# haosulab/ActiveZero

Hardware: AMD Instinct MI355X
Metric: stereo pairs/sec (540x960, D=192) fwd+bwd (higher is better)
Workload: dtype f32; 1 GPU; configs[1]: PSMNet 540x960 (padded to 544 rows) D=192 fwd+bwd+Adam, supervised disparity loss, batch 4 per GPU; global_batch=4, height=540, width=960, maxdisp=192, parallelism=dp1

## Files before the change

### activezero_amd/agg3d.py

```python
import torch

from . import bn2d, conv3d, costconv, ops


def _mode_of(conv):
    if isinstance(conv, torch.nn.ConvTranspose3d):
        return conv3d.DECONV_S2
    return conv3d.CONV_S1 if conv.stride[0] == 1 else conv3d.CONV_S2


def volume_from_features(feat_l, feat_r, ndisp, lazy=None):
    fl = feat_l.permute(0, 2, 3, 1).contiguous()
    fr = feat_r.permute(0, 2, 3, 1).contiguous()
    if lazy is None:
        lazy = not torch.is_grad_enabled()
    if lazy:
        return conv3d.LazyCostVolume(fl, fr, ndisp)
    return ops.cost_volume_ndhwc(fl, fr, ndisp)


def costvol_conv_bn(feat_l, feat_r, ndisp, unit, relu=False, arith=None):
    conv, bn = unit[0], unit[1]
    raw = costconv.costvol_conv(feat_l, feat_r, ndisp, conv.weight, arith)
    b, d, h, w, c = raw.shape
    y = bn2d.bn_act(raw.view(b, d * h, w, c).permute(0, 3, 1, 2), bn, relu=relu)
    return y.permute(0, 2, 3, 1).reshape(b, d, h, w, c)


def conv_bn(vol, unit, relu=False, add=None, arith=None, defer=None):
    return conv3d.conv_bn(vol, unit[0], unit[1], _mode_of(unit[0]), relu, add, arith, defer)


def deconv_bn(vol, unit, relu=False, add=None, arith=None):
    return conv3d.conv_bn(vol, unit[0], unit[1], conv3d.DECONV_S2, relu, add, arith)


def conv_logits(vol, conv, add=None, arith=None, affine=None):
    return conv3d.conv_logits(vol, conv, add, arith.sink if arith is not None else None, affine)


def add(a, b):
    return conv3d.add(a, b)


def fanout(x, n):
    return conv3d.fanout(x, n)
```

### activezero_amd/conv3d.py

```python
import collections
import os

import torch

from . import _lib, overlap, packing, profiler
from .amax import AMAX_SLOTS, ZEROS, absmax, _get_amax, _set_amax, weight_amax
from .handover import slot_contribute, slot_leftover, slot_register, sum_parts
from .ops import _call, _chk, _p, _stream

CONV_S1, CONV_S2, DECONV_S2 = 0, 1, 2
FP32, BF16X6, F16X3 = 0, 1, 3
_PREC = {"fp32": FP32, "bf16x6": BF16X6, "f16x3": F16X3}
_BWD_F16 = os.environ.get("AZ_BWD_F16", "1") != "0"
PRESPLIT = os.environ.get("AZ_PRESPLIT", "1") != "0"
BF16X6_R16 = 2
_ROLL = os.environ.get("AZ_CONV_ROLL", "1") != "0"


_OFF32 = 0xffffff00


def _fits32(x, cin, cout):
    if isinstance(x, LazyCostVolume):
        return True
# ... 322 lines not shown
    return _wgrad(dy, x, 1 if mode == CONV_S1 else 2, cout, cin, "conv", precision, sink)


def _presplit_ok(x, raw, mode, cin, cout, need_gx, need_gw):
    lib = _lib.lib()
    b, d, h, w, _ = raw.shape
    if need_gx:
        op, ci, co = _dgrad_launch(mode, cin, cout)[:3]
        if not _f16_launch_ok(op, ci, co, raw) or lib.az_conv3d_fwd_f16_split_ok(op, b, ci, co, d, h, w) != 1:
            return False
    if need_gw:
        if not _f16_wgrad_ok(mode, cin, cout):
            return False
        _, dx_, hx, wx, _ = x.shape
        if mode == DECONV_S2:
            ok, bit = lib.az_conv3d_wgrad_f16_split_ok(2, b, cin, cout, dx_, hx, wx, d, h, w), 2
        else:
            ok, bit = lib.az_conv3d_wgrad_f16_split_ok(1 if mode == CONV_S1 else 2, b, cout, cin, d, h, w, dx_, hx, wx), 1
        if not ok & bit:
            return False
    return bool(need_gx or need_gw)


class _ConvBN(torch.autograd.Function):

    @staticmethod
    def forward(ctx, x, weight, gamma, beta, residual, bn, mode, relu, arith, defer=None, x_slot=None, res_slot=None):
        ctx.x_slot, ctx.res_slot = x_slot, res_slot
        x = _chk(x, "x")
        if residual is not None:
            residual = _chk(residual, "residual")
        training = bn.training or not bn.track_running_stats
        eps = float(bn.eps)
        cin, cout = _fwd_launch(weight, mode)[:2]
        with torch.cuda.device(x.device):
            if not training:
                scale, shift = eval_affine(bn, x)
                raw = _conv(x, weight, mode, arith.conv)
                y = torch.empty_like(raw)
                y_amax = ZEROS.take(raw)
                _call("az_bn3d_apply", _p(y), _p(raw), _p(scale), _p(shift), _p(residual), int(relu),
                      raw.numel() // cout, cout, _p(y_amax), _stream())
                _set_amax(y, y_amax)
                ctx.save_for_backward(x, weight, gamma, raw, y if relu else None, bn.running_mean.clone(),
                                      scale, None, None)
                ctx.cfg = (mode, relu, residual is not None, cin, cout, arith, False)
                return y
            raw, part, cnt, ntiles = _conv(x, weight, mode, arith.conv, stats=True)
            scale, shift = x.new_empty(cout), x.new_empty(cout)
            mean, invstd = x.new_empty(cout), x.new_empty(cout)
            track = bn.track_running_stats and bn.running_mean is not None
            momentum = 0.1 if bn.momentum is None else float(bn.momentum)
            nbt = bn.num_batches_tracked if (track and bn.num_batches_tracked is not None) else None
            scratch = x.new_empty(int(_lib.lib().az_bn3d_finalize_scratch(cout))) if ntiles >= 4096 else None
            _call("az_bn3d_finalize", _p(mean), _p(invstd), _p(scale), _p(shift),
                  _p(bn.running_mean) if track else None, _p(bn.running_var) if track else None,
                  _p(part), _p(cnt), _p(gamma.detach()), _p(beta.detach()), ntiles, cout, eps,
                  momentum, _p(nbt), _p(scratch), scratch.numel() if scratch is not None else 0, _stream())
            if nbt is not None:
                packing.touched(nbt, bn.running_mean, bn.running_var)
            nvox = raw.numel() // cout
            if defer is not None and relu and residual is None:
                defer.scale, defer.shift = scale, shift
                y = raw
            else:
                y = torch.empty_like(raw)
                y_amax = ZEROS.take(raw)
                with profiler.scope(f"bn3d_apply_{cout}", bytes=4.0 * raw.numel() * (3 if residual is not None else 2),
                                    bound="hbm"):
                    _call("az_bn3d_apply", _p(y), _p(raw), _p(scale), _p(shift), _p(residual), int(relu),
                          nvox, cout, _p(y_amax), _stream())
                _set_amax(y, y_amax)
        remask = relu and residual is None
        ctx.save_for_backward(x, weight, gamma, raw, y if (relu and not remask) else None, mean, invstd,
                              scale if remask else None, shift if remask else None)
        if arith.sink is not None and not arith.sink.owns(weight):
            arith = arith._replace(sink=None)
        ctx.cfg = (mode, relu, residual is not None, cin, cout, arith, True)
        ctx.x_amax = _get_amax(x)
        return y

    @staticmethod
    def backward(ctx, gy):
# ... 11 lines not shown
                dgamma = (dz * (raw - rm)).sum(dim=(0, 1, 2, 3)) * rinv
                dx_raw = (dz * s_).contiguous()
                g_res = dz if has_res else None
            else:
                lib = _lib.lib()
                dx_raw = torch.empty_like(raw)
                dz = torch.empty_like(raw) if (has_res and relu) else None
                dgamma, dbeta = gy.new_empty(cout), gy.new_empty(cout)
                coef = gy.new_empty(cout, 3)
                ws_bytes = lib.az_bn3d_bwd_workspace(nvox, cout)
                ws = gy.new_empty(ws_bytes // 4)
                dx_amax = gy.new_empty(AMAX_SLOTS) if arith.bwd16 else None
                split = arith.bwd16 and PRESPLIT and _presplit_ok(x, raw, mode, cin, cout, ctx.needs_input_grad[0],
                                                                  ctx.needs_input_grad[1])
                with profiler.scope(f"bn3d_bwd_{cout}", bytes=4.0 * raw.numel() * (7 if (relu and y is not None) else 5), bound="hbm"):
                    _call("az_bn3d_bwd", _p(dx_raw), _p(dz), _p(dgamma), _p(dbeta), _p(coef), _p(ws), ws_bytes,
                          _p(gy), _p(y), _p(raw), _p(mean), _p(invstd), _p(gamma.detach()), _p(scale), _p(shift),
                          int(relu), nvox, cout, _p(dx_amax), int(split), _stream())
                if dx_amax is not None:
                    _set_amax(dx_raw, dx_amax)
                if split:
                    dx_raw.az_split = True
                g_res = (dz if relu else gy) if has_res else None
            gx = gw = None
            if has_res:
                g_res = slot_contribute(ctx.res_slot, plain=g_res)
            if ctx.needs_input_grad[0]:
                gx = slot_contribute(ctx.x_slot, make=lambda r: _input_grad(dx_raw, weight, mode, cin, cout,
                                                                             F16X3 if arith.bwd16 else arith.conv, r))
            if ctx.needs_input_grad[1]:
                if getattr(ctx, "x_amax", None) is not None and _get_amax(x) is None:
                    _set_amax(x, ctx.x_amax)
                gw = _weight_grad(x, dx_raw, mode, cin, cout, F16X3 if arith.bwd16 else arith.wgrad, arith.sink)
        return gx, gw, dgamma, dbeta, g_res, None, None, None, None, None, None, None


class DeferredAffine:

    def __init__(self):
        self.scale = self.shift = None

    @property
    def pending(self):
        return self.scale is not None


def conv_bn(x, conv, bn, mode, relu=False, residual=None, arith=None, defer=None):
    arith = _arith(arith)
    if isinstance(x, LazyCostVolume):
        if torch.is_grad_enabled() or bn.training:
            raise RuntimeError("LazyCostVolume is an inference-only operand")
        with torch.cuda.device(x.fl.device):
            scale, shift = eval_affine(bn, x.fl, cache=True)
            return _conv(x, conv.weight, mode, arith.conv, scale, shift, residual, relu, cache=True)
    training = bn.training or not bn.track_running_stats
    if not training and not torch.is_grad_enabled():
# ... 32 lines not shown
    def backward(ctx, g):
        x, w, scale, shift = ctx.saved_tensors
        g = _chk(g.contiguous(), "grad_logits")
        b, d, h, wd, _ = _dims(x)
        gx = gw = None
        with torch.cuda.device(g.device):
            if ctx.needs_input_grad[0]:
                gx = torch.empty_like(x)
                with profiler.scope("conv3d_c1_dgrad", bytes=4.0 * (x.numel() + g.numel()), bound="hbm"):
                    _call("az_conv3d_c1_dgrad", _p(gx), _p(g), _p(w), b, d, h, wd, _stream())
            if ctx.needs_input_grad[1]:
                gw = torch.empty_like(w)
                with overlap.scope(ctx.sink, x, g, gw, scale, shift), \
                        profiler.scope("conv3d_c1_wgrad", bytes=4.0 * (x.numel() + g.numel()), bound="hbm"):
                    _call("az_conv3d_c1_wgrad", _p(gw), _p(x), _p(g), _p(scale), _p(shift), b, d, h, wd, _stream())
        return gx, gw, (g if ctx.has_add else None), None, None, None


def conv_logits(x, conv, addend=None, sink=None, affine=None):
    sc, sh = (affine.scale, affine.shift) if (affine is not None and affine.pending) else (None, None)
    return _ConvLogits.apply(x, sink.weight(conv.weight) if sink is not None else conv.weight, addend, sink, sc, sh)


class _AddRelu(torch.autograd.Function):
    @staticmethod
    def forward(ctx, a, b):
        a, b = _chk(a, "a"), _chk(b, "b")
        y = torch.empty_like(a)
        y_amax = ZEROS.take(a)
        with torch.cuda.device(a.device):
            _call("az_add_relu", _p(y), _p(a), _p(b), 0, a.numel(), _p(y_amax), _stream())
        _set_amax(y, y_amax)
        return y

    @staticmethod
    def backward(ctx, g):
        return g, g


def add(a, b):
    return _AddRelu.apply(a, b)


class _FanOut(torch.autograd.Function):

    @staticmethod
# ... 27 lines not shown
```

### activezero_amd/csrc/az_conv3d_c1.hip

```cpp
#include "az_common.h"
#include "az_launch_math.h"

#define C1_TH 8
#define C1_TW 32
#define C1_VS 36
#define C1_GP 36
typedef float c1_f2 __attribute__((ext_vector_type(2)));
#define C1_FMA2(a, b, c) __builtin_elementwise_fma(a, b, c)


#define C1F_TH 8
#define C1F_TW 16
template <int CTRL>
__device__ __forceinline__ float c1_dpp_add(float v) {
    return v + __builtin_bit_cast(float, __builtin_amdgcn_update_dpp(0, __builtin_bit_cast(int, v), CTRL, 0xf, 0xf, true));
}
__global__ void __launch_bounds__(256)
c1_fwd_kernel(float *__restrict__ out, const float *__restrict__ in, const float *__restrict__ w,
              const float *__restrict__ addend, const float *__restrict__ in_scale,
              const float *__restrict__ in_shift, int D, int H, int W, int tiles_x, int dseg) {
    constexpr int SX = C1F_TW + 2, SY = C1F_TH + 2;
    __shared__ __attribute__((aligned(16))) float slab[SY * SX * C1_VS];
    const int tx0 = (blockIdx.x % tiles_x) * C1F_TW, ty0 = (blockIdx.x / tiles_x) * C1F_TH;
    const int d0 = blockIdx.y * dseg, d1 = min(d0 + dseg, D), b = blockIdx.z;
// ... 70 lines not shown
        const int od = id - 1;
        if (od >= d0 && od < d1) {
            float mine = 0.f;
#pragma unroll
            for (int j = 0; j < 8; ++j) {
                float v = a_prev[j][0] + a_prev[j][1];
                v = c1_dpp_add<0xB1>(v);
                v = c1_dpp_add<0x4E>(v);
                v = c1_dpp_add<0x141>(v);
                v = c1_dpp_add<0x140>(v);
                mine = (cp == j) ? v : mine;
            }
            const int ow = tx0 + lx0 + cp;
            if (cp < 8 && oh < H && ow < W) {
                const size_t o = (((size_t)b * D + od) * H + oh) * W + ow;
                out[o] = addend ? mine + addend[o] : mine;
            }
        }
#pragma unroll
        for (int j = 0; j < 8; ++j) { a_prev[j] = a_cur[j]; a_cur[j] = a_next[j]; a_next[j] = c1_f2{0.f, 0.f}; }
    }
}

__device__ __forceinline__ void c1_load_gtile(float *gt, const float *__restrict__ gout, int b,
                                              int od, int ty0, int tx0, int D, int H, int W) {
    constexpr int SX = C1_TW + 2, SY = C1_TH + 2;
    for (int q = threadIdx.x; q < 3 * SY * SX; q += 256) {
        const int sx = q % SX;
        const int r = q / SX;
        const int sy = r % SY, sd = r / SY;
        const int gd = od - 1 + sd, gh = ty0 - 1 + sy, gw = tx0 - 1 + sx;
        gt[r * C1_GP + sx] = (gd >= 0 && gd < D && gh >= 0 && gh < H && gw >= 0 && gw < W)
                                 ? gout[(((size_t)b * D + gd) * H + gh) * W + gw] : 0.f;
    }
}
__device__ __forceinline__ void c1_row6(float (&r)[6], const float *gt, int pd, int sy, int lx0) {
    const float *row = static_cast<const float *>(__builtin_assume_aligned(gt + (pd * (C1_TH + 2) + sy) * C1_GP + lx0, 16));
    const float4 a = *reinterpret_cast<const float4 *>(row);
    const float2 c = *reinterpret_cast<const float2 *>(row + 4);
    r[0] = a.x; r[1] = a.y; r[2] = a.z; r[3] = a.w; r[4] = c.x; r[5] = c.y;
}

__global__ void __launch_bounds__(256)
c1_dgrad_kernel(float *__restrict__ gin, const float *__restrict__ gout,
                const float *__restrict__ w, int D, int H, int W, int tiles_x) {
    constexpr int SY = C1_TH + 2;
    __shared__ __attribute__((aligned(16))) float gt[3 * SY * C1_GP];
    const int tx0 = (blockIdx.x % tiles_x) * C1_TW, ty0 = (blockIdx.x / tiles_x) * C1_TH;
    const int od = blockIdx.y, b = blockIdx.z;
    c1_load_gtile(gt, gout, b, od, ty0, tx0, D, H, W);
    const int cp = threadIdx.x & 15, grp = threadIdx.x >> 4;
    c1_f2 wp[27];
#pragma unroll
    for (int t = 0; t < 27; ++t) wp[t] = c1_f2{w[(cp * 2 + 0) * 27 + t], w[(cp * 2 + 1) * 27 + t]};
    __syncthreads();
#pragma unroll 1
    for (int p = 0; p < C1_TH * C1_TW / 128; ++p) {
// ... 94 lines not shown
                        const int t = (kd * 3 + kh) * 3 + kw;
#pragma unroll
                        for (int j = 0; j < 4; ++j) {
                            const c1_f2 g2 = {r[j + 2 - kw], r[j + 2 - kw]};
                            a01[t] = C1_FMA2(g2, x01[j], a01[t]);
                            a23[t] = C1_FMA2(g2, x23[j], a23[t]);
                        }
                    }
                }
        }
    }
#pragma unroll
    for (int c = 0; c < 4; ++c)
#pragma unroll
        for (int t = 0; t < 27; ++t) {
            float v = (c < 2 ? a01[t] : a23[t])[c & 1];
            v += __shfl_xor(v, 8); v += __shfl_xor(v, 16); v += __shfl_xor(v, 32);
            if ((threadIdx.x & 63) < 8) atomicAdd(&red[(quad * 4 + c) * 27 + t], v);
        }
    __syncthreads();
    for (int q = threadIdx.x; q < 864; q += 256) atomicAdd(&gw[q], red[q]);
}

static int c1_check(int B, int D, int H, int W) {
    if (!(B > 0 && D > 0 && H > 0 && W > 0)) return AZ_EINVAL;
    if (B > 65535 || D > 65535) return AZ_EUNSUPPORTED;
    return AZ_OK;
}

extern "C" int az_conv3d_c1_fwd(float *logits, const float *in, const float *w,
                                const float *addend, const float *in_scale, const float *in_shift, int B, int D,
                                int H, int W, void *stream) {
    AZ_REQUIRE_PTR(logits); AZ_REQUIRE_PTR(in); AZ_REQUIRE_PTR(w);
    if ((in_scale == nullptr) != (in_shift == nullptr)) return AZ_EINVAL;
    if (int e = c1_check(B, D, H, W)) return e;
    const int tiles_x = (W + C1F_TW - 1) / C1F_TW, tiles_y = (H + C1F_TH - 1) / C1F_TH;
    const int best = az_c1_fwd_dseg((long long)tiles_x * tiles_y * B, D);
    hipLaunchKernelGGL(c1_fwd_kernel, dim3(tiles_x * tiles_y, (D + best - 1) / best, B), dim3(256), 0,
                       az_stream(stream), logits, in, w, addend, in_scale, in_shift, D, H, W, tiles_x, best);
    return az_launch_status();
}

extern "C" int az_conv3d_c1_dgrad(float *grad_in, const float *grad_logits, const float *w,
                                  int B, int D, int H, int W, void *stream) {
    AZ_REQUIRE_PTR(grad_in); AZ_REQUIRE_PTR(grad_logits); AZ_REQUIRE_PTR(w);
    if (int e = c1_check(B, D, H, W)) return e;
    const int tiles_x = (W + C1_TW - 1) / C1_TW, tiles_y = (H + C1_TH - 1) / C1_TH;
    hipLaunchKernelGGL(c1_dgrad_kernel, dim3(tiles_x * tiles_y, D, B), dim3(256), 0,
                       az_stream(stream), grad_in, grad_logits, w, D, H, W, tiles_x);
    return az_launch_status();
}

extern "C" int az_conv3d_c1_wgrad(float *grad_w, const float *in, const float *grad_logits,
                                  const float *in_scale, const float *in_shift, int B, int D, int H, int W,
                                  void *stream) {
    AZ_REQUIRE_PTR(grad_w); AZ_REQUIRE_PTR(in); AZ_REQUIRE_PTR(grad_logits);
    if ((in_scale == nullptr) != (in_shift == nullptr)) return AZ_EINVAL;
    if (int e = c1_check(B, D, H, W)) return e;
    if (hipMemsetAsync(grad_w, 0, 864 * sizeof(float), az_stream(stream)) != hipSuccess)
        return AZ_ELAUNCH;
    const int tiles_x = (W + C1_TW - 1) / C1_TW, tiles_y = (H + C1_TH - 1) / C1_TH;
    const long long ntiles = az_c1_wgrad_tiles(B, D, H, W);
    const unsigned grid = (unsigned)az_c1_wgrad_grid(ntiles);
    hipLaunchKernelGGL(c1_wgrad_kernel, dim3(grid), dim3(256), 0, az_stream(stream), grad_w, in,
                       grad_logits, in_scale, in_shift, D, H, W, tiles_x, tiles_y, ntiles);
    return az_launch_status();
}

extern "C" int az_conv3d_c1_plan(long long *plan, int B, int D, int H, int W) {
    AZ_REQUIRE_PTR(plan);
    if (int e = c1_check(B, D, H, W)) return e;
    const long long patches = (long long)((W + C1F_TW - 1) / C1F_TW) * ((H + C1F_TH - 1) / C1F_TH) * B;
    const int dseg = az_c1_fwd_dseg(patches, D);
    const long long ntiles = az_c1_wgrad_tiles(B, D, H, W);
    plan[0] = dseg;
    plan[1] = patches * ((D + dseg - 1) / dseg);
    plan[2] = ntiles;
    plan[3] = az_c1_wgrad_grid(ntiles);
    return AZ_OK;
}
```

### activezero_amd/csrc/az_launch_math.h

```cpp
#pragma once
#if defined(__HIPCC__)
#define AZ_HD __host__ __device__ __forceinline__
#else
#define AZ_HD inline
#endif

AZ_HD int az_xcd_map(int bid, int nblk) {
    const int xcd = bid & 7, q8 = nblk >> 3, r8 = nblk & 7;
    return (xcd < r8 ? xcd * (q8 + 1) : r8 * (q8 + 1) + (xcd - r8) * q8) + (bid >> 3);
}

AZ_HD void az_conv_tile_decode(int lin, int map_mode, int band_rows, int tiles_x, int rows_y, int Dt, int &tix, int &tiy,
                               int &td, int &b) {
    tix = lin % tiles_x; lin /= tiles_x;
    if (map_mode >= 2) {
        const int per_b = Dt * rows_y;
        b = lin / per_b;
        int l = lin - b * per_b;
        const int full = (rows_y / band_rows) * band_rows * Dt;
        int band, rows;
        if (l < full) { band = l / (band_rows * Dt); l -= band * band_rows * Dt; rows = band_rows; }
        else { band = rows_y / band_rows; l -= full; rows = rows_y - band * band_rows; }
        td = l / rows;
        tiy = band * band_rows + (l - td * rows);
// ... 72 lines not shown
}

#define AZ_C1_FWD_SLOTS 768
inline long long az_c1_fwd_cost(long long patches, int D, int dseg) {
    const long long blocks = patches * ((D + dseg - 1) / dseg);
    return ((blocks + AZ_C1_FWD_SLOTS - 1) / AZ_C1_FWD_SLOTS) * (dseg + 2);
}
inline int az_c1_fwd_dseg(long long patches, int D) {
    int best = 1;
    long long best_cost = -1;
    for (int nseg = 1; nseg <= D; ++nseg) {
        const int dseg = (D + nseg - 1) / nseg;
        const long long cost = az_c1_fwd_cost(patches, D, dseg);
        if (best_cost < 0 || cost < best_cost) { best_cost = cost; best = dseg; }
    }
    return best;
}
#define AZ_C1_WGRAD_MAX_GRID 2048
inline long long az_c1_wgrad_tiles(int B, int D, int H, int W) {
    return (long long)B * D * ((H + 7) / 8) * ((W + 31) / 32);
}
inline int az_c1_wgrad_grid(long long ntiles) {
    return (int)(ntiles < AZ_C1_WGRAD_MAX_GRID ? ntiles : AZ_C1_WGRAD_MAX_GRID);
}

AZ_HD void az_roll_decode(int lin, int tiles_x, int tyb, int nseg, int &tix, int &tiy, int &seg, int &b) {
    tix = lin % tiles_x; lin /= tiles_x;
    tiy = lin % tyb; lin /= tyb;
    seg = lin % nseg;
    b = lin / nseg;
}

#define AZ_R_SY 10
#define AZ_R_SX 18
#define AZ_R_NQ (AZ_R_SY * AZ_R_SX * 8)
AZ_HD bool az_roll_piece(int tid, int it, int &sy, int &sx) {
    const int vox = (tid >> 3) + 32 * it;
    sy = vox / AZ_R_SX;
    sx = vox - sy * AZ_R_SX;
    return tid + 256 * it < AZ_R_NQ;
}

inline int az_wgrad16_workgroups(long long ncols, int slots, int ntiles, int cap) {
    int best = 1;
    double best_score = -1.0;
    const int step = 8 / (ntiles > 2 ? 4 : ntiles);
// ... 112 lines not shown
```

### activezero_amd/nets/psmnet/psmnet_3.py

```python
import math

from activezero_amd import overlap
from activezero_amd import agg3d, amax, conv3d, ops, packing
from activezero_amd.nets.psmnet.psmnet_submodule_3 import *
from activezero_amd.nets.psmnet import psmnet_submodule_3 as _sub


def _relu_unit(cin, cout, stride):
    return nn.Sequential(convbn_3d(cin, cout, kernel_size=3, stride=stride, pad=1),
                         nn.ReLU(inplace=True))


def _up_unit(cin, cout):
    return nn.Sequential(
        nn.ConvTranspose3d(cin, cout, kernel_size=3, padding=1, output_padding=1, stride=2,
                           bias=False),
        nn.BatchNorm3d(cout))


class hourglass(nn.Module):
    def __init__(self, inplanes):
        super().__init__()
        c2 = inplanes * 2
        self.conv1 = _relu_unit(inplanes, c2, 2)
# ... 53 lines not shown
        for m in self.modules():
            if isinstance(m, (nn.Conv2d, nn.Conv3d)):
                fan = m.out_channels * math.prod(m.kernel_size)
                m.weight.data.normal_(0, math.sqrt(2.0 / fan))
            elif isinstance(m, (nn.BatchNorm2d, nn.BatchNorm3d)):
                m.weight.data.fill_(1)
                m.bias.data.zero_()
            elif isinstance(m, nn.Linear):
                m.bias.data.zero_()

    def _aggregate(self, vol, first=None, arith=None):
        a = self.arith if arith is None else arith
        c0 = first if first is not None else agg3d.conv_bn(vol, self.dres0[0], relu=True, arith=a)
        c0 = agg3d.conv_bn(c0, self.dres0[2], relu=True, arith=a)
        t = agg3d.conv_bn(c0, self.dres1[0], relu=True, arith=a)
        c0 = agg3d.conv_bn(t, self.dres1[2], add=c0, arith=a)

        c0a, c0b, c0c, c0d = agg3d.fanout(c0, 4)
        out1, pre1, post1 = self.dres2(c0a, None, None, out_add=c0b, arith=a)
        out2, _pre2, post2 = self.dres3(out1, pre1, post1, out_add=c0c, arith=a)
        out3, _pre3, _post3 = self.dres4(out2, pre1, post2, out_add=c0d, arith=a)

        def head(cls, v, running):
            aff = conv3d.DeferredAffine() if (torch.is_grad_enabled() and cls[0][1].training) else None
            mid = agg3d.conv_bn(v, cls[0], relu=True, arith=a, defer=aff)
            return agg3d.conv_logits(mid, cls[2], running, arith=a, affine=aff)

        cost1 = head(self.classif1, out1, None)
        cost2 = head(self.classif2, out2, cost1)
        cost3 = head(self.classif3, out3, cost2)
        return cost1, cost2, cost3

    def _pass_arith(self, like):
        sink = overlap.begin(self, like) if self.wgrad_overlap else None
        if self.arith.conv == conv3d.F16X3 or self.arith.bwd16:
            ws = overlap.conv_weights(self)
            if torch.is_grad_enabled():
                packing.prepack(ws)
            amax.prime_weight_amax(ws)
        return self.arith._replace(sink=sink)

    def _from_features(self, feat_l, feat_r, arith=None):
        a = self.arith if arith is None else arith
        first = agg3d.costvol_conv_bn(feat_l, feat_r, self.maxdisp // 4, self.dres0[0], relu=True, arith=a)
        cost1, cost2, cost3 = self._aggregate(None, first, a)
        pred3 = ops.softargmin(cost3)
        if self.training:
            return pred3, ops.softargmin(cost2), ops.softargmin(cost1)
        return pred3
# ... 9 lines not shown
```

### activezero_amd/profiler.py

```python
import contextlib

import torch

PEAK = {"mfma": (157.3, "TFLOP/s"),
        "hbm": (8000.0, "GB/s")}

_active = False
_records = {}
_side_depth = 0
_side_pending = False


def side(delta):
    global _side_depth, _side_pending
    _side_depth += delta
    _side_pending = True


def joined():
    global _side_pending
    _side_pending = False


def start():
# ... 84 lines not shown
    data = json.load(open(clock_json))["kernels"]
    for sym in _PMC_NAMES[scope_name]:
        if sym in data:
            return dict(data[sym], kernel=sym, carried_from="profiles/" + os.path.basename(clock_json),
                        note="counter pass (tools/pmc_clock.sh) on another box; not measured in this run")
    return None


def _rate(r):
    peak, unit = PEAK[r["bound"]]
    basis = "fp32 MFMA dense" if r["bound"] == "mfma" else "HBM3E spec"
    if r.get("peak"):
        peak, basis = r["peak"]
    work = r["flops"] / 1e12 if r["bound"] == "mfma" else r["bytes"] / 1e9
    return work / (r["avg_ms"] * 1e-3), peak, basis, unit


_ROCPROF_FAMILY = [(r"^(conv|deconv)_wgrad_s1_", "conv3d_wgrad_r16_kernel"),
                   (r"^(conv|deconv)_wgrad_s2_", "conv3d_wgrad_s2r16_kernel"),
                   (r"^(conv3d|dgrad)_m0_(32|64)_32$", "conv3d_roll_kernel"),
                   (r"^(conv3d|dgrad)_m2_64_32$", "conv3d_t2roll_kernel"),
                   (r"^(conv3d|dgrad)_m1_", "conv3d_s2roll_kernel / conv3d_gather_kernel (stride 2)"),
                   (r"^(conv3d|dgrad)_m", "conv3d_gather_kernel"),
                   (r"^bn3d_bwd_", "bn_bwd_reduce_kernel + bn_bwd_apply_kernel (3-D)"),
                   (r"^bn2d_bwd", "bn_bwd_reduce_kernel + bn_bwd_apply_kernel (2-D)"),
                   (r"^bn3d_apply_", "bn_apply_kernel"),
                   (r"^conv2d_wgrad", "conv2d_wgrad_*"),
                   (r"^conv2d", "conv2d_*")]


def _family(scope_name):
    import re
    for pat, fam in _ROCPROF_FAMILY:
        if re.search(pat, scope_name):
            return fam
    return scope_name


def roofline(prof, pmc_json=None, clock_json=None, ms_per_step=None, steps=1, solo=None):
    if not prof:
        return None
    name, r = max(prof.items(), key=lambda kv: kv[1]["total_ms"])
    achieved, peak, peak_basis, unit = _rate(r)
    work_of = lambda v: v["flops"] / 1e12 if v["bound"] == "mfma" else v["bytes"] / 1e9
    out = {"kernel": name, "bound": r["bound"], "achieved": achieved, "peak": peak, "unit": unit, "frac": achieved / peak,
           "traffic": None}
# ... 75 lines not shown
```

### include/azhip.h

```cpp
#ifndef AZHIP_H
#define AZHIP_H

#include <stddef.h>
#include <stdint.h>

#ifdef __cplusplus
extern "C" {
#endif

#define AZ_OK 0
#define AZ_EINVAL (-1)
#define AZ_ENULL (-2)
#define AZ_ELAUNCH (-3)
#define AZ_EUNSUPPORTED (-4)
#define AZ_EWORKSPACE (-5)

const char *az_strerror(int code);
#define AZ_ABI_VERSION 6
int az_abi_version(void);
int az_option(const char *name);
int az_hbm_copy_probe(float *dst, const float *src, long long n, void *stream);

int az_warp_scatter(float *dst, const float *src, const int32_t *disp, int N, int C, int H,
                    int W, int sign, void *stream);
// ... 116 lines not shown
int az_conv2d_wgrad_bf16(float *grad_w, float *workspace, long long workspace_bytes, const float *grad_out,
                         const float *in, int B, int H, int W, int cm, int cn, int cm_real, int cn_real,
                         int go_cstride, int in_cstride, void *stream);
int az_conv2d_wgrad_f16(float *grad_w, float *workspace, long long workspace_bytes, const float *grad_out,
                        const float *in, const float *go_amax, const float *in_amax, int B, int H, int W,
                        int cm, int cn, int cm_real, int cn_real, int go_cstride, int in_cstride, int kh,
                        int kw, int dilation, void *stream);
int az_conv2d_roll_pack_f16(float *packed, const float *w, const float *w_amax, int cin, int cout,
                            long long stride_out, long long stride_in, int flip, void *stream);
int az_conv2d_roll_fwd_f16(float *out, const float *in, const float *packed, const float *in_amax,
                           const float *w_amax, const float *scale, const float *shift, const float *residual,
                           int relu, int B, int H, int W, int cin, int cout, void *stream);
int az_conv2d_roll_fwd_stats_f16(float *out, float *partials, float *counts, const float *in, const float *packed,
                                 const float *in_amax, const float *w_amax, int groups, int B, int H, int W,
                                 int cin, int cout, void *stream);

int az_conv3d_c1_fwd(float *logits, const float *in, const float *w, const float *addend,
                     const float *in_scale, const float *in_shift, int B, int D, int H, int W, void *stream);
int az_conv3d_c1_dgrad(float *grad_in, const float *grad_logits, const float *w, int B, int D,
                       int H, int W, void *stream);
int az_conv3d_c1_wgrad(float *grad_w, const float *in, const float *grad_logits, const float *in_scale,
                       const float *in_shift, int B, int D, int H, int W, void *stream);
int az_conv3d_c1_plan(long long *plan , int B, int D, int H, int W);

long long az_bn3d_finalize_scratch(int C);
int az_bn3d_finalize(float *mean, float *invstd, float *scale, float *shift,
                     float *running_mean, float *running_var, const float *partials,
                     const float *counts, const float *gamma, const float *beta,
                     long long ntiles, int C, float eps, float momentum,
                     long long *num_batches_tracked, float *scratch, long long scratch_floats, void *stream);
long long az_bn3d_stats_tiles(long long nvox, int C);
int az_bn3d_stats(float *partials, float *counts, const float *x, long long nvox, int C, void *stream);
long long az_bn2d_workspace(int groups, long long nvox, int C);
int az_bn2d_fwd(float *y, float *mean, float *invstd, float *scale, float *shift, float *running_mean,
                float *running_var, const float *x, const float *residual, const float *gamma,
                const float *beta, float *workspace, long long workspace_bytes, int relu, int groups,
                long long nvox, int C, float eps, float momentum, long long *num_batches_tracked ,
                const float *partials, const float *counts, long long partial_tiles ,
                float *y_amax , void *stream);
int az_bn2d_bwd(float *dx, float *dz_out, float *dgamma, float *dbeta, float *workspace,
                long long workspace_bytes, const float *dy, const float *y, const float *x,
                const float *mean, const float *invstd, const float *gamma, const float *scale,
                const float *shift, int relu, int groups, long long nvox, int C,
                float *dx_amax , void *stream);
int az_bn3d_eval_affine(float *scale, float *shift, const float *gamma, const float *beta,
                        const float *running_mean, const float *running_var, float eps, int C,
// ... 161 lines not shown
```

Measured before the change: 48.10 pairs/s.

## Fuse classifier head conv-BN-ReLU-logits backward into dedicated kernels

Adds a fused autograd path for the PSMNet classifier head (32->32 conv + BN + ReLU + 32->1 logits conv). It runs in the backward pass through three new kernels: sums, finalize and apply. These compute the logits dgrad, the ReLU mask, the BN reductions, the logits wgrad and the BN input grad together, without materialising the intermediate activated tensor and its gradient. The aim is to cut HBM traffic and launches on the large D×H×W×32 volumes. The cost is a more complex path that handles non-finite values through a separate slow accumulation route with atomics.

```diff
diff --git a/activezero_amd/agg3d.py b/activezero_amd/agg3d.py
--- a/activezero_amd/agg3d.py
+++ b/activezero_amd/agg3d.py
@@ -39,6 +39,10 @@
     return conv3d.conv_logits(vol, conv, add, arith.sink if arith is not None else None, affine)
 
 
+def head(vol, unit, conv, add=None, arith=None, fused=None):
+    return conv3d.head(vol, unit[0], unit[1], conv, add, arith, fused)
+
+
 def add(a, b):
     return conv3d.add(a, b)
 
diff --git a/activezero_amd/conv3d.py b/activezero_amd/conv3d.py
--- a/activezero_amd/conv3d.py
+++ b/activezero_amd/conv3d.py
@@ -368,6 +368,37 @@
     return bool(need_gx or need_gw)
 
 
+def _conv_batch_stats(x, weight, gamma, beta, bn, mode, precision):
+    cout = _fwd_launch(weight, mode)[1]
+    eps = float(bn.eps)
+    raw, part, cnt, ntiles = _conv(x, weight, mode, precision, stats=True)
+    scale, shift = x.new_empty(cout), x.new_empty(cout)
+    mean, invstd = x.new_empty(cout), x.new_empty(cout)
+    track = bn.track_running_stats and bn.running_mean is not None
+    momentum = 0.1 if bn.momentum is None else float(bn.momentum)
+    nbt = bn.num_batches_tracked if (track and bn.num_batches_tracked is not None) else None
+    scratch = x.new_empty(int(_lib.lib().az_bn3d_finalize_scratch(cout))) if ntiles >= 4096 else None
+    _call("az_bn3d_finalize", _p(mean), _p(invstd), _p(scale), _p(shift),
+          _p(bn.running_mean) if track else None, _p(bn.running_var) if track else None,
+          _p(part), _p(cnt), _p(gamma.detach()), _p(beta.detach()), ntiles, cout, eps,
+          momentum, _p(nbt), _p(scratch), scratch.numel() if scratch is not None else 0, _stream())
+    if nbt is not None:
+        packing.touched(nbt, bn.running_mean, bn.running_var)
+    return raw, mean, invstd, scale, shift
+
+
+def _layer_grads(ctx, x, weight, dx_raw, mode, cin, cout, arith):
+    gx = gw = None
+    if ctx.needs_input_grad[0]:
+        gx = slot_contribute(ctx.x_slot, make=lambda r: _input_grad(dx_raw, weight, mode, cin, cout,
+                                                                     F16X3 if arith.bwd16 else arith.conv, r))
+    if ctx.needs_input_grad[1]:
+        if getattr(ctx, "x_amax", None) is not None and _get_amax(x) is None:
+            _set_amax(x, ctx.x_amax)
+        gw = _weight_grad(x, dx_raw, mode, cin, cout, F16X3 if arith.bwd16 else arith.wgrad, arith.sink)
+    return gx, gw
+
+
 class _ConvBN(torch.autograd.Function):
 
     @staticmethod
@@ -377,7 +408,6 @@
         if residual is not None:
             residual = _chk(residual, "residual")
         training = bn.training or not bn.track_running_stats
-        eps = float(bn.eps)
         cin, cout = _fwd_launch(weight, mode)[:2]
         with torch.cuda.device(x.device):
             if not training:
@@ -392,19 +422,7 @@
                                       scale, None, None)
                 ctx.cfg = (mode, relu, residual is not None, cin, cout, arith, False)
                 return y
-            raw, part, cnt, ntiles = _conv(x, weight, mode, arith.conv, stats=True)
-            scale, shift = x.new_empty(cout), x.new_empty(cout)
-            mean, invstd = x.new_empty(cout), x.new_empty(cout)
-            track = bn.track_running_stats and bn.running_mean is not None
-            momentum = 0.1 if bn.momentum is None else float(bn.momentum)
-            nbt = bn.num_batches_tracked if (track and bn.num_batches_tracked is not None) else None
-            scratch = x.new_empty(int(_lib.lib().az_bn3d_finalize_scratch(cout))) if ntiles >= 4096 else None
-            _call("az_bn3d_finalize", _p(mean), _p(invstd), _p(scale), _p(shift),
-                  _p(bn.running_mean) if track else None, _p(bn.running_var) if track else None,
-                  _p(part), _p(cnt), _p(gamma.detach()), _p(beta.detach()), ntiles, cout, eps,
-                  momentum, _p(nbt), _p(scratch), scratch.numel() if scratch is not None else 0, _stream())
-            if nbt is not None:
-                packing.touched(nbt, bn.running_mean, bn.running_var)
+            raw, mean, invstd, scale, shift = _conv_batch_stats(x, weight, gamma, beta, bn, mode, arith.conv)
             nvox = raw.numel() // cout
             if defer is not None and relu and residual is None:
                 defer.scale, defer.shift = scale, shift
@@ -462,16 +480,9 @@
                 if split:
                     dx_raw.az_split = True
                 g_res = (dz if relu else gy) if has_res else None
-            gx = gw = None
             if has_res:
                 g_res = slot_contribute(ctx.res_slot, plain=g_res)
-            if ctx.needs_input_grad[0]:
-                gx = slot_contribute(ctx.x_slot, make=lambda r: _input_grad(dx_raw, weight, mode, cin, cout,
-                                                                             F16X3 if arith.bwd16 else arith.conv, r))
-            if ctx.needs_input_grad[1]:
-                if getattr(ctx, "x_amax", None) is not None and _get_amax(x) is None:
-                    _set_amax(x, ctx.x_amax)
-                gw = _weight_grad(x, dx_raw, mode, cin, cout, F16X3 if arith.bwd16 else arith.wgrad, arith.sink)
+            gx, gw = _layer_grads(ctx, x, weight, dx_raw, mode, cin, cout, arith)
         return gx, gw, dgamma, dbeta, g_res, None, None, None, None, None, None, None
 
 
@@ -550,6 +561,69 @@
     return _ConvLogits.apply(x, sink.weight(conv.weight) if sink is not None else conv.weight, addend, sink, sc, sh)
 
 
+HEAD_FUSED = os.environ.get("AZ_HEAD_FUSED", "1") != "0"
+
+
+class _Head(torch.autograd.Function):
+
+    @staticmethod
+    def forward(ctx, v, weight, gamma, beta, w1, addend, bn, arith, x_slot):
+        ctx.x_slot = x_slot
+        v = _chk(v, "x")
+        w1c = _chk(w1.detach().contiguous(), "weight")
+        if addend is not None:
+            addend = _chk(addend.contiguous(), "addend")
+        with torch.cuda.device(v.device):
+            raw, mean, invstd, scale, shift = _conv_batch_stats(v, weight, gamma, beta, bn, CONV_S1, arith.conv)
+            b, d, h, wd, _ = _dims(raw)
+            out = raw.new_empty(b, d, h, wd)
+            with profiler.scope("conv3d_c1_fwd", bytes=4.0 * (raw.numel() + out.numel()), bound="hbm"):
+                _call("az_conv3d_c1_fwd", _p(out), _p(raw), _p(w1c), _p(addend), _p(scale), _p(shift), b, d, h, wd, _stream())
+        ctx.save_for_backward(v, weight, gamma, beta, w1c, raw, mean, invstd, scale, shift)
+        if arith.sink is not None and not arith.sink.owns(weight):
+            arith = arith._replace(sink=None)
+        ctx.arith, ctx.has_add = arith, addend is not None
+        ctx.x_amax = _get_amax(v)
+        return out
+
+    @staticmethod
+    def backward(ctx, g):
+        v, weight, gamma, beta, w1, raw, mean, invstd, scale, shift = ctx.saved_tensors
+        arith = ctx.arith
+        g = _chk(g.contiguous(), "grad_logits")
+        b, d, h, wd, cout = _dims(raw)
+        with torch.cuda.device(g.device):
+            dx_raw, gw1 = torch.empty_like(raw), torch.empty_like(w1)
+            dgamma, dbeta, coef = g.new_empty(cout), g.new_empty(cout), g.new_empty(cout, 3)
+            ws_bytes = _lib.lib().az_conv3d_c1_head_bwd_workspace(b, d, h, wd)
+            ws = g.new_empty(ws_bytes // 4)
+            dx_amax = g.new_empty(AMAX_SLOTS) if arith.bwd16 else None
+            with profiler.scope("conv3d_c1_head_bwd", bytes=4.0 * (3 * raw.numel() + 2 * g.numel()), bound="hbm"):
+                _call("az_conv3d_c1_head_bwd", _p(dx_raw), _p(gw1), _p(dgamma), _p(dbeta), _p(coef), _p(ws), ws_bytes,
+                      _p(raw), _p(g), _p(w1), _p(mean), _p(invstd), _p(gamma.detach()), _p(scale), _p(shift),
+                      b, d, h, wd, _p(dx_amax), _stream())
+            if dx_amax is not None:
+                _set_amax(dx_raw, dx_amax)
+            gx, gw = _layer_grads(ctx, v, weight, dx_raw, CONV_S1, cout, cout, arith)
+        return gx, gw, dgamma, dbeta, gw1, (g if ctx.has_add else None), None, None, None
+
+
+def head(v, conv, bn, logits_conv, addend=None, arith=None, fused=None):
+    arith = _arith(arith)
+    fused = HEAD_FUSED if fused is None else bool(fused)
+    train = torch.is_grad_enabled() and bn.training
+    sink = arith.sink
+    if (fused and train and not isinstance(v, LazyCostVolume) and v.dim() == 5 and conv.stride[0] == 1
+            and tuple(conv.weight.shape) == (32, 32, 3, 3, 3) and tuple(logits_conv.weight.shape) == (1, 32, 3, 3, 3)
+            and _lib.lib().az_conv3d_c1_head_bwd_workspace(*v.shape[:4]) > 0):
+        w = sink.weight(conv.weight) if sink is not None else conv.weight
+        w1 = sink.weight(logits_conv.weight) if sink is not None else logits_conv.weight
+        return _Head.apply(v, w, bn.weight, bn.bias, w1, addend, bn, arith, slot_register(v))
+    aff = DeferredAffine() if train else None
+    mid = conv_bn(v, conv, bn, CONV_S1, relu=True, arith=arith, defer=aff)
+    return conv_logits(mid, logits_conv, addend, sink, aff)
+
+
 class _AddRelu(torch.autograd.Function):
     @staticmethod
     def forward(ctx, a, b):
diff --git a/activezero_amd/csrc/az_conv3d_c1.hip b/activezero_amd/csrc/az_conv3d_c1.hip
--- a/activezero_amd/csrc/az_conv3d_c1.hip
+++ b/activezero_amd/csrc/az_conv3d_c1.hip
@@ -116,17 +116,22 @@
     }
 }
 
-__device__ __forceinline__ void c1_load_gtile(float *gt, const float *__restrict__ gout, int b,
-                                              int od, int ty0, int tx0, int D, int H, int W) {
+template <bool CHK = false>
+__device__ __forceinline__ int c1_load_gtile(float *gt, const float *__restrict__ gout, int b,
+                                             int od, int ty0, int tx0, int D, int H, int W) {
     constexpr int SX = C1_TW + 2, SY = C1_TH + 2;
+    int bad = 0;
     for (int q = threadIdx.x; q < 3 * SY * SX; q += 256) {
         const int sx = q % SX;
         const int r = q / SX;
         const int sy = r % SY, sd = r / SY;
         const int gd = od - 1 + sd, gh = ty0 - 1 + sy, gw = tx0 - 1 + sx;
-        gt[r * C1_GP + sx] = (gd >= 0 && gd < D && gh >= 0 && gh < H && gw >= 0 && gw < W)
-                                 ? gout[(((size_t)b * D + gd) * H + gh) * W + gw] : 0.f;
-    }
+        const float v = (gd >= 0 && gd < D && gh >= 0 && gh < H && gw >= 0 && gw < W)
+                            ? gout[(((size_t)b * D + gd) * H + gh) * W + gw] : 0.f;
+        gt[r * C1_GP + sx] = v;
+        if (CHK) bad |= (__float_as_uint(v) & 0x7fffffffu) >= 0x7f800000u;
+    }
+    return bad;
 }
 __device__ __forceinline__ void c1_row6(float (&r)[6], const float *gt, int pd, int sy, int lx0) {
     const float *row = static_cast<const float *>(__builtin_assume_aligned(gt + (pd * (C1_TH + 2) + sy) * C1_GP + lx0, 16));
@@ -267,6 +272,261 @@
     for (int q = threadIdx.x; q < 864; q += 256) atomicAdd(&gw[q], red[q]);
 }
 
+__device__ __forceinline__ bool c1_finite(float x) { return (__float_as_uint(x) & 0x7fffffffu) < 0x7f800000u; }
+template <bool NT>
+__device__ __forceinline__ float2 c1_ld2(const float *p) {
+    if (NT) {
+        const c1_f2 v = __builtin_nontemporal_load(reinterpret_cast<const c1_f2 *>(p));
+        return make_float2(v[0], v[1]);
+    }
+    return *reinterpret_cast<const float2 *>(p);
+}
+__device__ __forceinline__ void c1_head_exc_voxel(float *__restrict__ exc, const float *gt, const float *__restrict__ w,
+                                                  int ly, int lx, int c, float x, float sc, float sh, float mu, float is) {
+    constexpr int SY = C1_TH + 2;
+    float gx = 0.f;
+#pragma unroll 1
+    for (int t = 0; t < 27; ++t) {
+        const int kd = t / 9, kh = (t / 3) % 3, kw = t % 3;
+        gx = fmaf(gt[((2 - kd) * SY + ly + 2 - kh) * C1_GP + lx + 2 - kw], w[c * 27 + t], gx);
+    }
+    const float y = fmaf(x, sc, sh), dz = y > 0.f ? gx : 0.f, a = az_relu(y);
+    atomicAdd(&exc[c * 29 + 0], dz);
+    atomicAdd(&exc[c * 29 + 1], dz * ((x - mu) * is));
+#pragma unroll 1
+    for (int t = 0; t < 27; ++t) {
+        const int kd = t / 9, kh = (t / 3) % 3, kw = t % 3;
+        atomicAdd(&exc[c * 29 + 2 + t], gt[((2 - kd) * SY + ly + 2 - kh) * C1_GP + lx + 2 - kw] * a);
+    }
+}
+
+template <bool NT>
+__global__ void __launch_bounds__(256)
+c1_head_sums_kernel(float *__restrict__ partial, float *__restrict__ exc, const float *__restrict__ raw,
+                    const float *__restrict__ gout, const float *__restrict__ w, const float *__restrict__ mean,
+                    const float *__restrict__ invstd, const float *__restrict__ scale, const float *__restrict__ shift,
+                    unsigned *__restrict__ amax_zero, int D, int H, int W, int tiles_x, int tiles_y, long long ntiles) {
+    constexpr int SY = C1_TH + 2;
+    __shared__ __attribute__((aligned(16))) float gt[3 * SY * C1_GP];
+    if (amax_zero && blockIdx.x == 0 && threadIdx.x < AZ_AMAX_SLOTS) amax_zero[threadIdx.x * AZ_AMAX_STRIDE] = 0u;
+    const int cp = threadIdx.x & 15, grp = threadIdx.x >> 4;
+    const float2 sc = reinterpret_cast<const float2 *>(scale)[cp], sh = reinterpret_cast<const float2 *>(shift)[cp];
+    const float2 mu = reinterpret_cast<const float2 *>(mean)[cp], is = reinterpret_cast<const float2 *>(invstd)[cp];
+    c1_f2 aM[27], aN[27];
+#pragma unroll
+    for (int t = 0; t < 27; ++t) { aM[t] = c1_f2{0.f, 0.f}; aN[t] = c1_f2{0.f, 0.f}; }
+    for (long long item = blockIdx.x; item < ntiles; item += gridDim.x) {
+        long long r_ = item;
+        const int tx0 = (int)(r_ % tiles_x) * C1_TW; r_ /= tiles_x;
+        const int ty0 = (int)(r_ % tiles_y) * C1_TH; r_ /= tiles_y;
+        const int od = (int)(r_ % D);
+        const int b = (int)(r_ / D);
+        __syncthreads();
+        const int bad = __syncthreads_or(c1_load_gtile<true>(gt, gout, b, od, ty0, tx0, D, H, W));
+#pragma unroll 1
+        for (int p = 0; p < C1_TH * C1_TW / 64; ++p) {
+            const int gi = p * 16 + grp, ly = gi >> 3, lx0 = (gi & 7) * 4;
+            const int ih = ty0 + ly;
+            const float *src = raw + ((((size_t)b * D + od) * H + ih) * W + tx0 + lx0) * 32 + cp * 2;
+            c1_f2 m2[4], n2[4];
+            unsigned excm = 0u;
+#pragma unroll
+            for (int j = 0; j < 4; ++j) {
+                const bool inb = ih < H && tx0 + lx0 + j < W;
+                float2 x = make_float2(0.f, 0.f);
+                if (inb) x = c1_ld2<NT>(src + j * 32);
+                const bool ok0 = c1_finite(x.x), ok1 = c1_finite(x.y);
+                const bool on0 = inb && !bad && ok0 && fmaf(x.x, sc.x, sh.x) > 0.f;
+                const bool on1 = inb && !bad && ok1 && fmaf(x.y, sc.y, sh.y) > 0.f;
+                m2[j] = c1_f2{on0 ? 1.f : 0.f, on1 ? 1.f : 0.f};
+                n2[j] = c1_f2{on0 ? (x.x - mu.x) * is.x : 0.f, on1 ? (x.y - mu.y) * is.y : 0.f};
+                if (inb && (bad || !ok0)) excm |= 1u << (2 * j);
+                if (inb && (bad || !ok1)) excm |= 2u << (2 * j);
+            }
+            if (excm != 0u) {
+#pragma unroll 1
+                for (int q = 0; q < 8; ++q)
+                    if ((excm >> q) & 1u) {
+                        const int e = q & 1;
+                        c1_head_exc_voxel(exc, gt, w, ly, lx0 + (q >> 1), cp * 2 + e, src[(q >> 1) * 32 + e], e ? sc.y : sc.x,
+                                          e ? sh.y : sh.x, e ? mu.y : mu.x, e ? is.y : is.x);
+                    }
+            }
+            if (bad) continue;
+#pragma unroll
+            for (int kd = 0; kd < 3; ++kd)
+#pragma unroll
+                for (int kh = 0; kh < 3; ++kh) {
+                    float r[6];
+                    c1_row6(r, gt, 2 - kd, ly + 2 - kh, lx0);
+#pragma unroll
+                    for (int kw = 0; kw < 3; ++kw) {
+                        const int t = (kd * 3 + kh) * 3 + kw;
+#pragma unroll
+                        for (int j = 0; j < 4; ++j) {
+                            const c1_f2 g2 = {r[j + 2 - kw], r[j + 2 - kw]};
+                            aM[t] = C1_FMA2(g2, m2[j], aM[t]);
+                            aN[t] = C1_FMA2(g2, n2[j], aN[t]);
+                        }
+                    }
+                }
+        }
+    }
+    const int wave = threadIdx.x >> 6, lane = threadIdx.x & 63;
+#pragma unroll
+    for (int k = 0; k < 7; ++k) {
+        __syncthreads();
+#pragma unroll
+        for (int a = 0; a < 16; ++a) {
+            const int idx = 16 * k + a;
+            if (idx < 108) {
+                float v = (idx < 54 ? aM[(idx % 54) >> 1] : aN[(idx % 54) >> 1])[idx & 1];
+                v += __shfl_xor(v, 16); v += __shfl_xor(v, 32);
+                if (lane < 16) gt[(a * 4 + wave) * 16 + cp] = v;
+            }
+        }
+        __syncthreads();
+        const int a = threadIdx.x >> 4, idx = 16 * k + a;
+        if (idx < 108) {
+            const float *q = &gt[a * 64 + cp];
+            const float s = (q[0] + q[16]) + (q[32] + q[48]);
+            const int set = idx / 54, t = (idx % 54) >> 1, e = idx & 1;
+            partial[(size_t)blockIdx.x * AZ_C1_HEAD_ROW + set * 864 + (cp * 2 + e) * 27 + t] = s;
+        }
+    }
+}
+
+__global__ void __launch_bounds__(1024)
+c1_head_finalize_kernel(float *__restrict__ dgamma, float *__restrict__ dbeta, float *__restrict__ coef,
+                        float *__restrict__ gw, const float *__restrict__ partial, const float *__restrict__ exc,
+                        int nrows, const float *__restrict__ w, const float *__restrict__ gamma,
+                        const float *__restrict__ mean, const float *__restrict__ invstd,
+                        const float *__restrict__ scale, const float *__restrict__ shift, double nvox) {
+    const int c = blockIdx.x, j = threadIdx.x & 63, r = threadIdx.x >> 6;
+    __shared__ double part[16][54];
+    __shared__ double col[54];
+    if (j < 54) {
+        const float *p = partial + (j < 27 ? c * 27 + j : 864 + c * 27 + j - 27);
+        double a = 0.0;
+        for (int row = r; row < nrows; row += 16) a += (double)p[(size_t)row * AZ_C1_HEAD_ROW];
+        part[r][j] = a;
+    }
+    __syncthreads();
+    if (threadIdx.x < 54) {
+        double s = 0.0;
+#pragma unroll
+        for (int k = 0; k < 16; ++k) s += part[k][threadIdx.x];
+        col[threadIdx.x] = s;
+    }
+    __syncthreads();
+    if (threadIdx.x < 27) {
+        const double a = (double)scale[c] / (double)invstd[c], b = (double)mean[c] * (double)scale[c] + (double)shift[c];
+        gw[c * 27 + threadIdx.x] = (float)(a * col[27 + threadIdx.x] + b * col[threadIdx.x] + (double)exc[c * 29 + 2 + threadIdx.x]);
+    }
+    if (threadIdx.x == 64) {
+        double sa = 0.0, sb = 0.0;
+        for (int t = 0; t < 27; ++t) {
+            sa += (double)w[c * 27 + t] * col[t];
+            sb += (double)w[c * 27 + t] * col[27 + t];
+        }
+        sa += (double)exc[c * 29 + 0];
+        sb += (double)exc[c * 29 + 1];
+        dbeta[c] = (float)sa;
+        dgamma[c] = (float)sb;
+        coef[c * 3 + 0] = gamma[c] * invstd[c];
+        coef[c * 3 + 1] = (float)(sa / nvox);
+        coef[c * 3 + 2] = (float)(sb / nvox);
+    }
+}
+
+template <bool NT>
+__global__ void __launch_bounds__(256)
+c1_head_apply_kernel(float *__restrict__ dx, const float *__restrict__ raw, const float *__restrict__ gout,
+                     const float *__restrict__ w, const float *__restrict__ mean, const float *__restrict__ invstd,
+                     const float *__restrict__ scale, const float *__restrict__ shift, const float *__restrict__ coef,
+                     unsigned *__restrict__ amax, int D, int H, int W, int tiles_x) {
+    constexpr int SY = C1_TH + 2;
+    __shared__ __attribute__((aligned(16))) float gt[3 * SY * C1_GP];
+    const int tx0 = (blockIdx.x % tiles_x) * C1_TW, ty0 = (blockIdx.x / tiles_x) * C1_TH;
+    const int od = blockIdx.y, b = blockIdx.z;
+    const int cp = threadIdx.x & 15, grp = threadIdx.x >> 4;
+    const size_t plane = (((size_t)b * D + od) * H * W) * 32 + cp * 2;
+    auto load = [&](int p, float2 (&x)[8]) {
+        const int gi = p * 16 + grp, oh = ty0 + (gi >> 2), ow = tx0 + (gi & 3) * 8;
+        const float *src = raw + plane + ((size_t)oh * W + ow) * 32;
+#pragma unroll
+        for (int j = 0; j < 8; ++j) {
+            x[j] = make_float2(0.f, 0.f);
+            if (oh < H && ow + j < W) x[j] = c1_ld2<NT>(src + j * 32);
+        }
+    };
+    float2 xa[8], xb[8];
+    load(0, xa);
+    c1_load_gtile(gt, gout, b, od, ty0, tx0, D, H, W);
+    c1_f2 wp[27];
+#pragma unroll
+    for (int t = 0; t < 27; ++t) wp[t] = c1_f2{w[(cp * 2 + 0) * 27 + t], w[(cp * 2 + 1) * 27 + t]};
+    const float2 sc = reinterpret_cast<const float2 *>(scale)[cp], sh = reinterpret_cast<const float2 *>(shift)[cp];
+    const float2 mu = reinterpret_cast<const float2 *>(mean)[cp], is = reinterpret_cast<const float2 *>(invstd)[cp];
+    const float k0x = coef[cp * 6 + 0], k1x = coef[cp * 6 + 1], k2x = coef[cp * 6 + 2];
+    const float k0y = coef[cp * 6 + 3], k1y = coef[cp * 6 + 4], k2y = coef[cp * 6 + 5];
+    unsigned am = 0;
+    __syncthreads();
+    auto pass = [&](int p, const float2 (&xr)[8]) {
+        const int gi = p * 16 + grp, ly = gi >> 2, lx0 = (gi & 3) * 8;
+        const int oh = ty0 + ly;
+        c1_f2 acc[8];
+#pragma unroll
+        for (int j = 0; j < 8; ++j) acc[j] = c1_f2{0.f, 0.f};
+#pragma unroll
+        for (int kd = 0; kd < 3; ++kd)
+#pragma unroll
+            for (int kh = 0; kh < 3; ++kh) {
+                float r[12];
+                {
+                    const float *row = static_cast<const float *>(__builtin_assume_aligned(
+                        gt + ((2 - kd) * SY + ly + 2 - kh) * C1_GP + lx0, 16));
+                    const float4 a = *reinterpret_cast<const float4 *>(row);
+                    const float4 c = *reinterpret_cast<const float4 *>(row + 4);
+                    const float2 e = *reinterpret_cast<const float2 *>(row + 8);
+                    r[0] = a.x; r[1] = a.y; r[2] = a.z; r[3] = a.w; r[4] = c.x; r[5] = c.y; r[6] = c.z; r[7] = c.w;
+                    r[8] = e.x; r[9] = e.y;
+                }
+#pragma unroll
+                for (int kw = 0; kw < 3; ++kw) {
+                    const int t = (kd * 3 + kh) * 3 + kw;
+#pragma unroll
+                    for (int j = 0; j < 8; ++j) {
+                        const c1_f2 g2 = {r[j + 2 - kw], r[j + 2 - kw]};
+                        acc[j] = C1_FMA2(g2, wp[t], acc[j]);
+                    }
+                }
+            }
+#pragma unroll
+        for (int j = 0; j < 8; ++j) asm volatile("" : "+v"(acc[j]));
+        if (oh < H) {
+            float *dst = dx + plane + ((size_t)oh * W + tx0 + lx0) * 32;
+#pragma unroll
+            for (int j = 0; j < 8; ++j)
+                if (tx0 + lx0 + j < W) {
+                    const float gx_ = fmaf(xr[j].x, sc.x, sh.x) > 0.f ? acc[j][0] : 0.f;
+                    const float gy_ = fmaf(xr[j].y, sc.y, sh.y) > 0.f ? acc[j][1] : 0.f;
+                    float2 o;
+                    o.x = k0x * (gx_ - k1x - (xr[j].x - mu.x) * is.x * k2x);
+                    o.y = k0y * (gy_ - k1y - (xr[j].y - mu.y) * is.y * k2y);
+                    if (NT) __builtin_nontemporal_store(c1_f2{o.x, o.y}, reinterpret_cast<c1_f2 *>(dst + j * 32));
+                    else *reinterpret_cast<float2 *>(dst + j * 32) = o;
+                    am = max(am, max(az_finite_abs_bits(o.x), az_finite_abs_bits(o.y)));
+                }
+        }
+    };
+    static_assert(C1_TH * C1_TW / 128 == 2, "two passes per tile");
+    load(1, xb);
+    pass(0, xa);
+    pass(1, xb);
+    if (amax) az_amax_flush(amax, am);
+}
+
 static int c1_check(int B, int D, int H, int W) {
     if (!(B > 0 && D > 0 && H > 0 && W > 0)) return AZ_EINVAL;
     if (B > 65535 || D > 65535) return AZ_EUNSUPPORTED;
@@ -312,6 +572,49 @@
     return az_launch_status();
 }
 
+extern "C" long long az_conv3d_c1_head_bwd_workspace(int B, int D, int H, int W) {
+    if (int e = c1_check(B, D, H, W)) return e;
+    return az_c1_head_workspace_floats(az_c1_wgrad_tiles(B, D, H, W)) * (long long)sizeof(float);
+}
+
+extern "C" int az_conv3d_c1_head_bwd(float *dx_raw, float *grad_w, float *dgamma, float *dbeta, float *coef,
+                                     float *workspace, long long workspace_bytes, const float *raw,
+                                     const float *grad_logits, const float *w, const float *mean, const float *invstd,
+                                     const float *gamma, const float *scale, const float *shift,
+                                     int B, int D, int H, int W, float *dx_amax, void *stream) {
+    AZ_REQUIRE_PTR(dx_raw); AZ_REQUIRE_PTR(grad_w); AZ_REQUIRE_PTR(dgamma); AZ_REQUIRE_PTR(dbeta); AZ_REQUIRE_PTR(coef);
+    AZ_REQUIRE_PTR(workspace); AZ_REQUIRE_PTR(raw); AZ_REQUIRE_PTR(grad_logits); AZ_REQUIRE_PTR(w); AZ_REQUIRE_PTR(mean);
+    AZ_REQUIRE_PTR(invstd); AZ_REQUIRE_PTR(gamma);
+    if ((scale == nullptr) != (shift == nullptr)) return AZ_EINVAL;
+    AZ_REQUIRE_PTR(scale);
+    if (int e = c1_check(B, D, H, W)) return e;
+    const long long ntiles = az_c1_wgrad_tiles(B, D, H, W);
+    if (workspace_bytes < az_c1_head_workspace_floats(ntiles) * (long long)sizeof(float)) return AZ_EWORKSPACE;
+    hipStream_t s = az_stream(stream);
+    const int tiles_x = (W + C1_TW - 1) / C1_TW, tiles_y = (H + C1_TH - 1) / C1_TH;
+    const int grid = az_c1_head_grid(ntiles);
+    float *exc = workspace + (size_t)grid * AZ_C1_HEAD_ROW;
+    if (hipMemsetAsync(exc, 0, AZ_C1_HEAD_EXC * sizeof(float), s) != hipSuccess) return AZ_ELAUNCH;
+    const double nvox = (double)B * D * H * W;
+    const bool nt = nvox * 32 * 4 >= (double)(256LL << 20);
+    unsigned *const am = reinterpret_cast<unsigned *>(dx_amax);
+    if (nt)
+        hipLaunchKernelGGL(c1_head_sums_kernel<true>, dim3(grid), dim3(256), 0, s, workspace, exc, raw, grad_logits, w, mean,
+                           invstd, scale, shift, am, D, H, W, tiles_x, tiles_y, ntiles);
+    else
+        hipLaunchKernelGGL(c1_head_sums_kernel<false>, dim3(grid), dim3(256), 0, s, workspace, exc, raw, grad_logits, w, mean,
+                           invstd, scale, shift, am, D, H, W, tiles_x, tiles_y, ntiles);
+    hipLaunchKernelGGL(c1_head_finalize_kernel, dim3(32), dim3(1024), 0, s, dgamma, dbeta, coef, grad_w,
+                       (const float *)workspace, (const float *)exc, grid, w, gamma, mean, invstd, scale, shift, nvox);
+    if (nt)
+        hipLaunchKernelGGL(c1_head_apply_kernel<true>, dim3(tiles_x * tiles_y, D, B), dim3(256), 0, s, dx_raw, raw,
+                           grad_logits, w, mean, invstd, scale, shift, (const float *)coef, am, D, H, W, tiles_x);
+    else
+        hipLaunchKernelGGL(c1_head_apply_kernel<false>, dim3(tiles_x * tiles_y, D, B), dim3(256), 0, s, dx_raw, raw,
+                           grad_logits, w, mean, invstd, scale, shift, (const float *)coef, am, D, H, W, tiles_x);
+    return az_launch_status();
+}
+
 extern "C" int az_conv3d_c1_plan(long long *plan, int B, int D, int H, int W) {
     AZ_REQUIRE_PTR(plan);
     if (int e = c1_check(B, D, H, W)) return e;
diff --git a/activezero_amd/csrc/az_launch_math.h b/activezero_amd/csrc/az_launch_math.h
--- a/activezero_amd/csrc/az_launch_math.h
+++ b/activezero_amd/csrc/az_launch_math.h
@@ -118,6 +118,15 @@
 }
 inline int az_c1_wgrad_grid(long long ntiles) {
     return (int)(ntiles < AZ_C1_WGRAD_MAX_GRID ? ntiles : AZ_C1_WGRAD_MAX_GRID);
+}
+#define AZ_C1_HEAD_MAX_GRID 768
+#define AZ_C1_HEAD_ROW 1728
+#define AZ_C1_HEAD_EXC 928
+inline int az_c1_head_grid(long long ntiles) {
+    return (int)(ntiles < AZ_C1_HEAD_MAX_GRID ? ntiles : AZ_C1_HEAD_MAX_GRID);
+}
+inline long long az_c1_head_workspace_floats(long long ntiles) {
+    return (long long)az_c1_head_grid(ntiles) * AZ_C1_HEAD_ROW + AZ_C1_HEAD_EXC;
 }
 
 AZ_HD void az_roll_decode(int lin, int tiles_x, int tyb, int nseg, int &tix, int &tiy, int &seg, int &b) {
diff --git a/activezero_amd/nets/psmnet/psmnet_3.py b/activezero_amd/nets/psmnet/psmnet_3.py
--- a/activezero_amd/nets/psmnet/psmnet_3.py
+++ b/activezero_amd/nets/psmnet/psmnet_3.py
@@ -99,9 +99,7 @@
         out3, _pre3, _post3 = self.dres4(out2, pre1, post2, out_add=c0d, arith=a)
 
         def head(cls, v, running):
-            aff = conv3d.DeferredAffine() if (torch.is_grad_enabled() and cls[0][1].training) else None
-            mid = agg3d.conv_bn(v, cls[0], relu=True, arith=a, defer=aff)
-            return agg3d.conv_logits(mid, cls[2], running, arith=a, affine=aff)
+            return agg3d.head(v, cls[0], cls[2], running, arith=a)
 
         cost1 = head(self.classif1, out1, None)
         cost2 = head(self.classif2, out2, cost1)
diff --git a/activezero_amd/profiler.py b/activezero_amd/profiler.py
--- a/activezero_amd/profiler.py
+++ b/activezero_amd/profiler.py
@@ -130,6 +130,7 @@
                    (r"^(conv3d|dgrad)_m2_64_32$", "conv3d_t2roll_kernel"),
                    (r"^(conv3d|dgrad)_m1_", "conv3d_s2roll_kernel / conv3d_gather_kernel (stride 2)"),
                    (r"^(conv3d|dgrad)_m", "conv3d_gather_kernel"),
+                   (r"^conv3d_c1_head_bwd$", "c1_head_sums_kernel + c1_head_finalize_kernel + c1_head_apply_kernel"),
                    (r"^bn3d_bwd_", "bn_bwd_reduce_kernel + bn_bwd_apply_kernel (3-D)"),
                    (r"^bn2d_bwd", "bn_bwd_reduce_kernel + bn_bwd_apply_kernel (2-D)"),
                    (r"^bn3d_apply_", "bn_apply_kernel"),
diff --git a/include/azhip.h b/include/azhip.h
--- a/include/azhip.h
+++ b/include/azhip.h
@@ -162,6 +162,12 @@
 int az_conv3d_c1_wgrad(float *grad_w, const float *in, const float *grad_logits, const float *in_scale,
                        const float *in_shift, int B, int D, int H, int W, void *stream);
 int az_conv3d_c1_plan(long long *plan , int B, int D, int H, int W);
+long long az_conv3d_c1_head_bwd_workspace(int B, int D, int H, int W);
+int az_conv3d_c1_head_bwd(float *dx_raw, float *grad_w, float *dgamma, float *dbeta, float *coef, float *workspace,
+                          long long workspace_bytes, const float *raw, const float *grad_logits, const float *w,
+                          const float *mean, const float *invstd, const float *gamma,
+                          const float *scale, const float *shift, int B, int D, int H, int W, float *dx_amax,
+                          void *stream);
 
 long long az_bn3d_finalize_scratch(int C);
 int az_bn3d_finalize(float *mean, float *invstd, float *scale, float *shift,
```

After: 48.47 pairs/s, median of 6. No clear change (+0.8%).
